# lanl-ansi/RestartSQP

Measured on NVIDIA B200. Metric: QP subproblems/sec, higher is better.
Workload: dtype f64

## Files before the change

restartsqp_b200/csrc/qp_kernel.cuh:

```cuda
#pragma once
#include <cuda_runtime.h>
#include <stdint.h>
#include "tma.cuh"

namespace sqpb200 {

#define QP_EPS 2.221e-16
#define QP_INFTY 1.0e20
#define QP_ZERO 1.0e-25
#define QP_BOUND_RELAX 1.0e4
#define QP_EPS_NUM (-1.0e3 * QP_EPS)
#define QP_EPS_DEN (1.0e3 * QP_EPS)
#define QP_EPS_FLIP (1.0e3 * QP_EPS)
#define QP_EPS_REG (1.0e3 * QP_EPS)
#define QP_EPS_LI (1.0e5 * QP_EPS)

enum { ST_OPTIMAL = 20, ST_INTERNAL = 21, ST_INFEASIBLE = 22, ST_UNBOUNDED = 23, ST_NOTINIT = 25, ST_HOMOTOPY = 28,
       ST_CAPACITY = 31  };
enum { MODE_COLD = 0, MODE_HOT_FIXED = 1, MODE_HOT_VARIED = 2,
       MODE_REINIT = 3  };
enum { FLAG_FLIPPING = 1, FLAG_RAMPING = 2, FLAG_DRIFT = 4, FLAG_KEEP_STATE = 8,
       FLAG_FORCE_GUESS = 16 ,
       FLAG_NO_CARRY = 32  };

// ... 60 lines not shown
    a.oW = o; if (a.large) o += a.cap * a.ld;
    if (a.large) o = (o + 15) & ~15;
    a.slice_doubles = o;
    a.state_doubles = a.oP + 2 * nV * nV;
    int p = 0;
    a.pAp = p; p += nV + 1; a.pAi = p; p += a.zA; a.pArp = p; p += nC + 1; a.pAci = p; p += a.zA; a.pAperm = p; p += a.zA;
    a.pHp = p; p += nV + 1; a.pHi = p; p += a.zH;
    a.pat_shorts = (p + 3) & ~3;
}

#ifdef __CUDACC__

__shared__ QPKernelArgs sA;
extern __shared__ __align__(128) double qp_smem[];

struct MinKey {
    double t;
    int pos;
};
__device__ __forceinline__ bool key_less(double t1, int p1, double t2, int p2) { return t1 < t2 || (t1 == t2 && p1 < p2); }

__device__ __forceinline__ double quot(double x, double d, double ri) {
    const double q0 = x * ri;
    const double r = __fma_rn(-q0, d, x);
    return __fma_rn(r, ri, q0);
}

#define QP_FN __noinline__
#define QP_U1 _Pragma("unroll 1")
#ifdef QP_PROFILE
#define PROF_T0 long long prof_t0_ = clock64();
#define PROF_RESET prof_t0_ = clock64();
#define PROF2_T0 long long prof_t2_ = clock64();
#define PROF2_ADD(i) do { long long t_ = clock64(); if (lane == 0 && sA.prof) atomicAdd((unsigned long long*)&sA.prof[i], (unsigned long long)(t_ - prof_t2_)); prof_t2_ = t_; } while (0)
#define PROF_ADD(i) do { long long t_ = clock64(); if (lane == 0 && sA.prof) atomicAdd((unsigned long long*)&sA.prof[i], (unsigned long long)(t_ - prof_t0_)); prof_t0_ = t_; } while (0)
#else
#define PROF_T0
#define PROF_RESET
#define PROF2_T0
#define PROF2_ADD(i) do { } while (0)
#define PROF_ADD(i) do { } while (0)
#endif
enum { PR_STEPDIR = 0, PR_RATIO = 1, PR_STEP = 2, PR_REMOVE = 3, PR_EXTEND = 4, PR_WVEC = 5, PR_ADD = 6, PR_REFAC_W = 7, PR_REFAC_M = 8,
       PR_REFAC_CHOL = 9, PR_DRIFT = 10, PR_ENSURE_LI = 11, PR_RSOLVE = 12, PR_SETUP = 13, PR_EPILOGUE = 14, PR_TOTAL = 15 };

template <int TEAM> struct PatIdx { typedef int type; };
template <> struct PatIdx<32> { typedef short type; };
template <> struct PatIdx<16> { typedef short type; };
template <> struct PatIdx<8> { typedef short type; };
template <int TEAM> __device__ __forceinline__ unsigned team_mask() {
    if (TEAM >= 32) return 0xffffffffu;
    return ((1u << (TEAM & 31)) - 1u) << ((threadIdx.x & 31) & ~(TEAM - 1));
}
__shared__ double* sSlice;
__shared__ int sClusterSize;
__shared__ uint32_t sPhase;
__shared__ __align__(8) uint64_t sFull[3];
__shared__ double sRedT[32];
__shared__ int sRedP[32];

#define QP_CTX                                                                                     \
    const int lane = (TEAM <= 32) ? (int)(threadIdx.x & (TEAM - 1)) : (int)threadIdx.x;            \
    double* const slice = (TEAM <= 32) ? qp_smem + (size_t)(threadIdx.x / TEAM) * sA.slice_doubles : sSlice; \
    int* const hdr = reinterpret_cast<int*>(slice);                                                \
    const int nV = sA.nV, nC = sA.nC, ld = sA.ld, cap = sA.cap;                                    \
    (void)lane; (void)hdr; (void)nV; (void)nC; (void)ld; (void)cap;
#define QP_PAT                                                                                     \
    const pidx* const pat = (TEAM <= 32)                                                           \
        ? reinterpret_cast<const pidx*>(qp_smem + (size_t)(blockDim.x / TEAM) * sA.slice_doubles) \
        : reinterpret_cast<const pidx*>(sA.gpat);

#define V_(name) (slice + sA.o##name)
#define S_(k) (reinterpret_cast<short*>(slice + sA.oS) + (k))
#define sB_ S_(0)
#define FR_ S_(nV)
#define posFR_ S_(2 * nV)
#define sC_ S_(3 * nV)
#define AC_ S_(3 * nV + nC)
#define posAC_ S_(3 * nV + 2 * nC)
#define R_(a_, b_) RT[(a_) * ld + (b_)]
#define T_(i, j) RT[(cap - 1 - (i)) * ld + (j)]
#define DOT_UNROLL _Pragma("unroll (TEAM <= 32 ? 1 : 8)")
#define SYNC() do { if (TEAM <= 32) __syncwarp(team_mask<TEAM>()); else __syncthreads(); } while (0)

template <int TEAM>
struct QPT {
    typedef typename PatIdx<TEAM>::type pidx;
    static __device__ __forceinline__ double H_row(const pidx* pat, const double* Hv, const double* v, int c) {
        const pidx *Hp = pat + sA.pHp, *Hi = pat + sA.pHi;
        const double reg = sA.is_lp ? QP_EPS_REG : 0.0;
        double s = 0.0;
        if (sA.has_H && !sA.is_lp) {
            int e1 = Hp[c + 1];
            QP_U1 for (int e = Hp[c]; e < e1; e++) s += Hv[e] * v[Hi[e]];
        }
        if (reg != 0.0) s += reg * v[c];
        return s;
    }
    static __device__ __forceinline__ double A_row(const pidx* pat, const double* Av, const double* v, int r) {
        const pidx *Arp = pat + sA.pArp, *Aci = pat + sA.pAci, *Aperm = pat + sA.pAperm;
        double s = 0.0;
        int k1 = Arp[r + 1];
        QP_U1 for (int k = Arp[r]; k < k1; k++) s += Av[Aperm[k]] * v[Aci[k]];
        return s;
    }
    static __device__ __forceinline__ double AT_col(const pidx* pat, const double* Av, const double* yc, int c) {
        const pidx *Ap = pat + sA.pAp, *Ai = pat + sA.pAi;
        double s = 0.0;
        int e1 = Ap[c + 1];
        QP_U1 for (int e = Ap[c]; e < e1; e++) s += Av[e] * yc[Ai[e]];
        return s;
    }
    static __device__ QP_FN void mulH(const double* v, double* out) {
        QP_CTX QP_PAT
        const double* Hv = V_(Hv);
        QP_U1 for (int c = lane; c < nV; c += TEAM) out[c] = H_row(pat, Hv, v, c);
        SYNC();
    }
    static __device__ QP_FN void mulH_noreg(const double* v, double* out) {
        QP_CTX QP_PAT
        const pidx *Hp = pat + sA.pHp, *Hi = pat + sA.pHi;
        const double* Hv = V_(Hv);
        const bool has_H = sA.has_H && !sA.is_lp;
        QP_U1 for (int c = lane; c < nV; c += TEAM) {
            double s = 0.0;
            if (has_H) {
                int e1 = Hp[c + 1];
                QP_U1 for (int e = Hp[c]; e < e1; e++) s += Hv[e] * v[Hi[e]];
            }
            out[c] = s;
        }
        SYNC();
    }
    static __device__ QP_FN void mulA(const double* v, double* out) {
        QP_CTX QP_PAT
        const double* Av = V_(Av);
        QP_U1 for (int r = lane; r < nC; r += TEAM) out[r] = A_row(pat, Av, v, r);
        SYNC();
    }
    static __device__ QP_FN void mulAT(const double* yc, double* out) {
        QP_CTX QP_PAT
        const double* Av = V_(Av);
        QP_U1 for (int c = lane; c < nV; c += TEAM) out[c] = AT_col(pat, Av, yc, c);
        SYNC();
    }
    static __device__ __forceinline__ double A_entry(const pidx* pat, const double* Av, int r, int c) {
        const pidx *Arp = pat + sA.pArp, *Aci = pat + sA.pAci, *Aperm = pat + sA.pAperm;
        double s = 0.0;
        int k1 = Arp[r + 1];
        QP_U1 for (int k = Arp[r]; k < k1; k++)
            if (Aci[k] == c) s += Av[Aperm[k]];
        return s;
    }

    static __device__ __forceinline__ MinKey team_min(double t, int pos) {
        const unsigned tm = team_mask<TEAM>();
        QP_U1 for (int o = (TEAM < 32 ? TEAM : 32) / 2; o > 0; o >>= 1) {
            double t2_ = __shfl_xor_sync(tm, t, o);
            int p2 = __shfl_xor_sync(tm, pos, o);
            if (key_less(t2_, p2, t, pos)) { t = t2_; pos = p2; }
        }
        if (TEAM > 32) {
            __syncthreads();
            if ((threadIdx.x & 31) == 0) { sRedT[threadIdx.x >> 5] = t; sRedP[threadIdx.x >> 5] = pos; }
            __syncthreads();
            t = sRedT[0]; pos = sRedP[0];
            QP_U1 for (int k = 1; k < TEAM / 32; k++)
                if (key_less(sRedT[k], sRedP[k], t, pos)) { t = sRedT[k]; pos = sRedP[k]; }
        }
        MinKey r; r.t = t; r.pos = pos;
        return r;
    }

    static __device__ __forceinline__ void givens(double a_, double b_, double& c, double& s, double& r) {
        if (a_ == 0.0) { c = 1.0; s = 0.0; r = b_; return; }
        double h = sqrt(a_ * a_ + b_ * b_);
        c = b_ / h; s = a_ / h; r = h;
    }

    static __device__ QP_FN void proj_column(int b) {
        QP_CTX
        double *t1 = V_(t1), *t2 = V_(t2);
        const double* Q = V_(Q);
        const short* posFR = posFR_;
        QP_U1 for (int i = lane; i < nV; i += TEAM) { int p = posFR[i]; t1[i] = (p >= 0) ? Q[p * ld + b] : 0.0; }
        SYNC();
        mulH(t1, t2);
    }
    static __device__ QP_FN int recompute_R() {
        QP_CTX
        const int nFR = hdr[0], nAC = hdr[1], nZ = nFR - nAC;
        if (nZ <= 0) return 0;
        double* RT = V_(RT);
        if (sA.is_lp) {
            double sr = sqrt(QP_EPS_REG);
            QP_U1 for (int k = lane; k < nZ * nZ; k += TEAM) { int a_ = k / nZ, b_ = k % nZ; R_(a_, b_) = (a_ == b_) ? sr : 0.0; }
            if constexpr (TEAM > 32) {
                double* W = V_(W);
                for (int k = lane; k < nZ * 64; k += TEAM) { const int a_ = k >> 6, c_ = k & 63; if (c_ < ld) W[(size_t)a_ * ld + c_] = (c_ == (a_ & 63)) ? 1.0 / sr : 0.0; }
            }
            SYNC();
            return 0;
        }
        if constexpr (TEAM > 32) return recompute_R_blocked();
        PROF_T0
        {
            QP_PAT
            const double *Q = V_(Q), *Hv = V_(Hv);
            double* Wc = V_(t1);
            const short *FR = FR_, *posFR = posFR_;
            const pidx *Hp = pat + sA.pHp, *Hi = pat + sA.pHi;
            const bool has_H = sA.has_H != 0;
            int CH = sA.nW / nFR;
            if (CH > nZ) CH = nZ;
            QP_U1 for (int b0 = 0; b0 < nZ; b0 += CH) {
                const int cw = (nZ - b0 < CH) ? nZ - b0 : CH;
                QP_U1 for (int e = lane; e < nFR * cw; e += TEAM) {
                    const int p = e / cw, bb = e - p * cw;
                    double s = 0.0;
                    if (has_H) {
                        const int c = FR[p], e1 = Hp[c + 1];
                        QP_U1 for (int h = Hp[c]; h < e1; h++) {
                            const int pr = posFR[Hi[h]];
                            s += Hv[h] * ((pr >= 0) ? Q[pr * ld + b0 + bb] : 0.0);
                        }
                    }
                    Wc[e] = s;
                }
                SYNC();
                QP_U1 for (int e = lane; e < (b0 + cw) * cw; e += TEAM) {
                    const int a_ = e / cw, bb = e - a_ * cw;
                    if (a_ <= b0 + bb) {
                        double s = 0.0;
                        QP_U1 for (int p = 0; p < nFR; p++) s += Q[p * ld + a_] * Wc[p * cw + bb];
                        R_(a_, b0 + bb) = s;
                    }
                }
                SYNC();
            }
        }
        PROF_ADD(PR_REFAC_M);
        QP_U1 for (int i = 0; i < nZ; i++) {
            QP_U1 for (int j = i + lane; j < nZ; j += TEAM) {
                double s = R_(i, j);
                DOT_UNROLL for (int k = 0; k < i; k++) s -= R_(k, i) * R_(k, j);
                R_(i, j) = s;
            }
            SYNC();
            double d = R_(i, i);
            SYNC();
            if (!(d > QP_ZERO)) return 1 + i;
            double dd = sqrt(d);
            QP_U1 for (int j = i + lane; j < nZ; j += TEAM) R_(i, j) = (j == i) ? dd : R_(i, j) / dd;
            QP_U1 for (int j = lane; j < i; j += TEAM) R_(i, j) = 0.0;
            SYNC();
        }
        PROF_ADD(PR_REFAC_CHOL);
        return 0;
    }

    static constexpr int LT_KC = 32, LT_STAGES = 3, LT_LD = 68, LT_NB = 64;
    static constexpr int LT_STAGE_DOUBLES = LT_KC * LT_LD;
    static constexpr int LT_D_LD = 65;
    static constexpr int LS_X = 0, LS_Y = LT_STAGES * LT_STAGE_DOUBLES, LS_D = 2 * LT_STAGES * LT_STAGE_DOUBLES,
                         LS_DI = LS_D + LT_NB * LT_D_LD, LS_RED = LS_DI + LT_NB * LT_D_LD, LS_TV = LS_RED + 8 * LT_NB,
                         LS_TOTAL = LS_TV + 2 * LT_NB;

    static __device__ __forceinline__ void large_sync() {
        asm volatile("fence.proxy.async;" ::: "memory");
        if (sClusterSize > 1) asm volatile("barrier.cluster.arrive.release.aligned;\n\tbarrier.cluster.wait.acquire.aligned;" ::: "memory");
        else __syncthreads();
    }
    static __device__ __forceinline__ void dmma(double (&c)[2], double a, double b) {
        asm volatile("mma.sync.aligned.m8n8k4.row.col.f64.f64.f64.f64 {%0,%1}, {%2}, {%3}, {%0,%1};" : "+d"(c[0]), "+d"(c[1]) : "d"(a), "d"(b));
    }
    template <int SIGN, bool TRI>
    static __device__ __forceinline__ void mma_tile(const double* X, int xw, const double* Y, int yw, int K, double* C, int na, int nb,
                                                    int ld, bool init_zero, int ga, int gb) {
        static_assert(TEAM == 512, "tile mapping assumes 16 warps");
        uint32_t ph = sPhase;
        double* Xs = qp_smem + LS_X;
        double* Ys = qp_smem + LS_Y;
        const int tid = threadIdx.x, warp = tid >> 5, l = tid & 31, g = l >> 2, t = l & 3;
        const int ra = (warp >> 2) * 16, cb = (warp & 3) * 16;
        double acc[2][2][2];
#pragma unroll
        for (int mi = 0; mi < 2; mi++)
#pragma unroll
            for (int ni = 0; ni < 2; ni++)
#pragma unroll
                for (int j = 0; j < 2; j++) {
                    const int a = ra + mi * 8 + g, b = cb + ni * 8 + t * 2 + j;
                    acc[mi][ni][j] = (!init_zero && a < na && b < nb && (!TRI || ga + a <= gb + b)) ? C[a * ld + b] : 0.0;
                }
        const int nch = (K + LT_KC - 1) / LT_KC;
        auto issue = [&](int chunk, int s) {
            const int rows = (K - chunk * LT_KC < LT_KC) ? K - chunk * LT_KC : LT_KC;
            if (l == 0) mbar_expect_tx(&sFull[s], (uint32_t)rows * (uint32_t)(xw + yw) * 8u);
            __syncwarp();
            if (l < rows) {
                const size_t kr = (size_t)(chunk * LT_KC + l) * ld;
                bulk_g2s(Xs + s * LT_STAGE_DOUBLES + l * LT_LD, X + kr, (uint32_t)xw * 8u, &sFull[s]);
                bulk_g2s(Ys + s * LT_STAGE_DOUBLES + l * LT_LD, Y + kr, (uint32_t)yw * 8u, &sFull[s]);
            }
        };
        if (warp == 0)
            for (int c = 0; c < LT_STAGES && c < nch; c++) issue(c, c);
        for (int c = 0; c < nch; c++) {
            const int s = c % LT_STAGES;
            while (!mbar_try_wait(&sFull[s], (ph >> s) & 1u)) {}
            ph ^= 1u << s;
            const int rows = (K - c * LT_KC < LT_KC) ? K - c * LT_KC : LT_KC;
            const double* xs = Xs + s * LT_STAGE_DOUBLES + ra + g;
            const double* ys = Ys + s * LT_STAGE_DOUBLES + cb + g;
            const int k4n = (rows + 3) >> 2;
#pragma unroll 2
            for (int k4 = 0; k4 < k4n; k4++) {
                const int kr = k4 * 4 + t;
                double a0 = xs[kr * LT_LD], a1 = xs[kr * LT_LD + 8], b0 = ys[kr * LT_LD], b1 = ys[kr * LT_LD + 8];
                if (kr >= rows) { a0 = 0.0; a1 = 0.0; b0 = 0.0; b1 = 0.0; }
                if (SIGN < 0) { a0 = -a0; a1 = -a1; }
                dmma(acc[0][0], a0, b0); dmma(acc[0][1], a0, b1); dmma(acc[1][0], a1, b0); dmma(acc[1][1], a1, b1);
            }
            __syncthreads();
            if (warp == 0 && c + LT_STAGES < nch) issue(c + LT_STAGES, s);
        }
#pragma unroll
        for (int mi = 0; mi < 2; mi++)
#pragma unroll
// ... 658 lines not shown
    }
    static __device__ QP_FN void bwd_solve_R_blocked(double* z, int n) {
        QP_CTX
        const double* RT = V_(RT);
        const double* W = V_(W);
        double* tv = qp_smem + LS_TV;
        const int tid = threadIdx.x, warp = tid >> 5, l = tid & 31;
        for (int i0 = ((n - 1) >> 6) << 6; i0 >= 0; i0 -= LT_NB) {
            const int nb = (n - i0 < LT_NB) ? n - i0 : LT_NB, i1 = i0 + nb;
            double dreg[4][2];
#pragma unroll
            for (int q = 0; q < 4; q++) {
                const int r = warp + (TEAM / 32) * q;
#pragma unroll
                for (int h = 0; h < 2; h++) { const int cc = r + l + 32 * h; dreg[q][h] = (r < nb && cc < nb) ? W[(size_t)(i0 + r) * ld + cc] : 0.0; }
            }
            {
                double s4[4] = {0.0, 0.0, 0.0, 0.0};
#pragma unroll 2
                for (int k = i1 + 2 * l; k < n; k += 64) {
                    const double zk = z[k], zk1 = (k + 1 < n) ? z[k + 1] : 0.0;
#pragma unroll
                    for (int q = 0; q < 4; q++) {
                        const int r = warp + (TEAM / 32) * q;
                        if (r < nb) { const double2 v = *reinterpret_cast<const double2*>(&R_(i0 + r, k)); s4[q] += v.x * zk + ((k + 1 < n) ? v.y * zk1 : 0.0); }
                    }
                }
#pragma unroll
                for (int q = 0; q < 4; q++) {
                    double sq = s4[q];
#pragma unroll
                    for (int o = 16; o > 0; o >>= 1) sq += __shfl_xor_sync(0xffffffffu, sq, o);
                    const int r = warp + (TEAM / 32) * q;
                    if (l == 0 && r < nb) tv[r] = z[i0 + r] - sq;
                }
            }
            __syncthreads();
#pragma unroll
            for (int q = 0; q < 4; q++) {
                const int r = warp + (TEAM / 32) * q;
                double s = 0.0;
#pragma unroll
                for (int h = 0; h < 2; h++) { const int cc = r + l + 32 * h; if (r < nb && cc < nb) s += dreg[q][h] * tv[cc]; }
#pragma unroll
                for (int o = 16; o > 0; o >>= 1) s += __shfl_xor_sync(0xffffffffu, s, o);
                if (l == 0 && r < nb) z[i0 + r] = s;
            }
            __syncthreads();
        }
    }
    static __device__ QP_FN void extend_Dinv(int b, double rho) {
        QP_CTX
        const double* RT = V_(RT);
        double* W = V_(W);
        const int i0 = (b >> 6) << 6, c = b - i0, tid = threadIdx.x;
        if (tid < c) {
            double s = 0.0;
            for (int q = tid; q < c; q++) s += W[(size_t)(i0 + tid) * ld + q] * R_(i0 + q, b);
            W[(size_t)(i0 + tid) * ld + c] = -s / rho;
        } else if (tid == c) W[(size_t)(i0 + c) * ld + c] = 1.0 / rho;
        __syncthreads();
    }
    static __device__ QP_FN int extend_R(int check_curvature) {
        QP_CTX
        const int nFR = hdr[0], nAC = hdr[1], nZ = nFR - nAC, b = nZ - 1;
        double *RT = V_(RT), *w = V_(w);
        if (sA.is_lp) {
            QP_U1 for (int a_ = lane; a_ < b; a_ += TEAM) { R_(a_, b) = 0.0; R_(b, a_) = 0.0; }
            if (lane == 0) R_(b, b) = sqrt(QP_EPS_REG);
            SYNC();
            if constexpr (TEAM > 32) extend_Dinv(b, sqrt(QP_EPS_REG));
            return 1;
        }
        const double *Q = V_(Q), *t2 = V_(t2);
        const short* FR = FR_;
        proj_column(b);
        if constexpr (TEAM > 32) {
            double* tmp = V_(a);
            for (int p = lane; p < nFR; p += TEAM) tmp[p] = t2[FR[p]];
            SYNC();
            col_sums_auto(sA.oQ, nFR, 0, b + 1, sA.oa, sA.ow, false);
        } else
        {
        QP_U1 for (int a_ = lane; a_ <= b; a_ += TEAM) {
            double s = 0.0;
            DOT_UNROLL for (int p = 0; p < nFR; p++) s += Q[p * ld + a_] * t2[FR[p]];
            w[a_] = s;
        }
        SYNC();
        }
        if constexpr (TEAM > 32) fwd_solve_R_blocked(w, b, b);
        else {
        double* rinv = V_(dy);
        QP_U1 for (int k = lane; k < b; k += TEAM) rinv[k] = 1.0 / R_(k, k);
        SYNC();
        QP_U1 for (int k = 0; k < b; k++) {
            double rk = quot(w[k], R_(k, k), rinv[k]);
            SYNC();
            if (lane == 0) R_(k, b) = rk;
            QP_U1 for (int i = k + 1 + lane; i < b; i += TEAM) w[i] -= R_(k, i) * rk;
            SYNC();
        }
        }
        double rho2 = w[b];
        if constexpr (TEAM > 32) {
            double part = 0.0;
            for (int k = lane; k < b; k += TEAM) part += R_(k, b) * R_(k, b);
            rho2 -= team_sum(part);
        } else
        {
        DOT_UNROLL for (int k = 0; k < b; k++) rho2 -= R_(k, b) * R_(k, b);
        }
        int ok = check_curvature ? (rho2 > QP_EPS_FLIP) : (rho2 > QP_ZERO);
        SYNC();
        if (!ok) return 0;
        if (lane == 0) R_(b, b) = sqrt(rho2);
        QP_U1 for (int a_ = lane; a_ < b; a_ += TEAM) R_(b, a_) = 0.0;
        SYNC();
        if constexpr (TEAM > 32) extend_Dinv(b, sqrt(rho2));
        return 1;
    }

    static __device__ QP_FN void constraint_w(int c, double& wz2, double& a2) {
        QP_CTX QP_PAT
        const int nFR = hdr[0], nAC = hdr[1], nZ = nFR - nAC;
        double *a = V_(a), *w = V_(w);
        const double *Q = V_(Q), *Av = V_(Av);
        const short* FR = FR_;
        QP_U1 for (int p = lane; p < nFR; p += TEAM) a[p] = A_entry(pat, Av, c, FR[p]);
        SYNC();
        if constexpr (TEAM > 32) {
            col_sums_auto(sA.oQ, nFR, 0, nFR, sA.oa, sA.ow, false);
            double s2p = 0.0, z2p = 0.0;
            for (int p = lane; p < nFR; p += TEAM) s2p += a[p] * a[p];
            for (int j = lane; j < nZ; j += TEAM) z2p += w[j] * w[j];
            a2 = team_sum(s2p); wz2 = team_sum(z2p);
            SYNC();
            return;
        }
        QP_U1 for (int j = lane; j < nFR; j += TEAM) {
            double s = 0.0;
            DOT_UNROLL for (int p = 0; p < nFR; p++) s += Q[p * ld + j] * a[p];
            w[j] = s;
        }
        SYNC();
        double s2 = 0.0, z2 = 0.0;
        DOT_UNROLL for (int p = 0; p < nFR; p++) s2 += a[p] * a[p];
        DOT_UNROLL for (int j = 0; j < nZ; j++) z2 += w[j] * w[j];
        wz2 = z2; a2 = s2;
        SYNC();
    }
    static __device__ QP_FN double rotation_chain(int cnt) {
        QP_CTX
        double *t2 = V_(t2), *t3 = V_(t3);
        const double* w = V_(w);
        QP_U1 for (int j = lane; j + 1 < cnt; j += TEAM) {
            double S = w[0] * w[0];
            bool anyprev = false;
            DOT_UNROLL for (int k = 1; k <= j; k++) { anyprev = anyprev || (w[k - 1] != 0.0); S = S + w[k] * w[k]; }
            const double a = anyprev ? sqrt(S) : w[j];
            if (a == 0.0) { t2[j] = 1.0; t3[j] = 0.0; }
            else { const double h = sqrt(S + w[j + 1] * w[j + 1]); t2[j] = w[j + 1] / h; t3[j] = a / h; }
        }
        double r;
        {
            const int j = cnt - 1;
            double S = w[0] * w[0];
            bool anyprev = false;
            DOT_UNROLL for (int k = 1; k <= j; k++) { anyprev = anyprev || (w[k - 1] != 0.0); S = S + w[k] * w[k]; }
            r = anyprev ? sqrt(S) : w[j];
        }
        SYNC();
        return r;
    }
    static __device__ QP_FN void add_constraint(int c, int status, bool carry_R = false) {
        QP_CTX
        const int nFR = hdr[0], nAC = hdr[1], nZ = nFR - nAC;
        double *Q = V_(Q), *RT = V_(RT);
        const double *t2 = V_(t2), *t3 = V_(t3), *w = V_(w);
        double r = rotation_chain(nZ);
        if constexpr (TEAM > 32) {
            rot_rows_auto(sA.oQ, nFR, nZ, sA.ot2, sA.ot3);
            if (carry_R) update_R_after_add(nZ);
        } else
        {
        QP_U1 for (int p = lane; p < nFR; p += TEAM) {
            double* q = Q + p * ld;
            double qa = q[0];
            QP_U1 for (int j = 0; j + 1 < nZ; j++) {
                double cs = t2[j], sn = t3[j], qb = q[j + 1];
                q[j] = cs * qa - sn * qb;
                qa = sn * qa + cs * qb;
            }
            if (nZ > 0) q[nZ - 1] = qa;
        }
        }
        QP_U1 for (int j = lane; j < nFR; j += TEAM) T_(nAC, j) = (j > nZ - 1) ? w[j] : ((j == nZ - 1) ? r : 0.0);
        if (lane == 0) { AC_[nAC] = (short)c; posAC_[c] = (short)nAC; sC_[c] = (short)status; hdr[1] = nAC + 1; }
        SYNC();
    }
    static __device__ QP_FN void removal_chain_regs(int i0, int c0) {
        QP_CTX
        const int nFR = hdr[0], nAC = hdr[1];
        double *Q = V_(Q), *RT = V_(RT), *t2 = V_(t2), *t3 = V_(t3);
        const unsigned tm = team_mask<TEAM>();
        constexpr int W = TEAM <= 32 ? TEAM : 32;
        const bool own = lane >= i0 && lane < nAC;
        double tb = own ? T_(lane, c0 - i0 + 1) : 0.0;
        QP_U1 for (int i = i0; i < nAC; i++) {
            const int cL = c0 - i;
            const bool act = own && lane >= i;
            const double ta = act ? T_(lane, cL) : 0.0;
            double cs, sn, r;
            givens(__shfl_sync(tm, ta, i, W), __shfl_sync(tm, tb, i, W), cs, sn, r);
            if (act) {
                T_(lane, cL + 1) = sn * ta + cs * tb;
                tb = cs * ta - sn * tb;
                if (lane == i) { T_(lane, cL) = 0.0; t2[i - i0] = cs; t3[i - i0] = sn; }
            }
        }
        SYNC();
        QP_U1 for (int p = lane; p < nFR; p += TEAM) {
            double* q = Q + p * ld;
            double qb = q[c0 - i0 + 1];
            QP_U1 for (int i = i0; i < nAC; i++) {
                const int cL = c0 - i;
                const double cs = t2[i - i0], sn = t3[i - i0], qa = q[cL];
                q[cL + 1] = sn * qa + cs * qb;
                qb = cs * qa - sn * qb;
            }
            q[c0 - nAC + 1] = qb;
        }
    }
    static __device__ QP_FN void remove_constraint(int c) {
        QP_CTX
        const int nFR = hdr[0], nAC = hdr[1];
        double *Q = V_(Q), *RT = V_(RT);
        short *AC = AC_, *posAC = posAC_;
        const int k = posAC[c];
        SYNC();
        if (TEAM <= 32 && nAC <= TEAM) {
            if (k + 1 < nAC) removal_chain_regs(k + 1, nFR - 1);
        } else {
        QP_U1 for (int i = k + 1; i < nAC; i++) {
            int cL = nFR - 1 - i;
            double cs, sn, r;
            givens(T_(i, cL), T_(i, cL + 1), cs, sn, r);
            SYNC();
            QP_U1 for (int ii = i + lane; ii < nAC; ii += TEAM) {
                double ta = T_(ii, cL), tb = T_(ii, cL + 1);
                T_(ii, cL) = (ii == i) ? 0.0 : cs * ta - sn * tb;
                T_(ii, cL + 1) = sn * ta + cs * tb;
            }
            if constexpr (TEAM > 32) {
                if (lane == 0) { V_(t2)[i - k - 1] = cs; V_(t3)[i - k - 1] = -sn; }
            } else
            {
            QP_U1 for (int p = lane; p < nFR; p += TEAM) {
                double qa = Q[p * ld + cL], qb = Q[p * ld + cL + 1];
                Q[p * ld + cL] = cs * qa - sn * qb;
                Q[p * ld + cL + 1] = sn * qa + cs * qb;
            }
            }
            SYNC();
        }
        }
        if constexpr (TEAM > 32) rot_rows_auto(sA.oQ, nFR, nAC - k, sA.ot2, sA.ot3, nFR - 1 - k, -1);
        QP_U1 for (int j = lane; j < nFR; j += TEAM)
            QP_U1 for (int i = k + 1; i < nAC; i++) T_(i - 1, j) = T_(i, j);
        SYNC();
        if (lane == 0) {
            QP_U1 for (int i = k + 1; i < nAC; i++) { AC[i - 1] = AC[i]; posAC[AC[i - 1]] = (short)(i - 1); }
            sC_[c] = 0; posAC[c] = -1; hdr[1] = nAC - 1;
        }
        SYNC();
    }
    static __device__ QP_FN double bound_w(int v) {
        QP_CTX
        const int nFR = hdr[0], nAC = hdr[1], nZ = nFR - nAC, p = posFR_[v];
        double* w = V_(w);
        const double* Q = V_(Q);
        QP_U1 for (int j = lane; j < nFR; j += TEAM) w[j] = Q[p * ld + j];
        SYNC();
        if constexpr (TEAM > 32) {
            double z2p = 0.0;
            for (int j = lane; j < nZ; j += TEAM) z2p += w[j] * w[j];
            const double z2s = team_sum(z2p);
            SYNC();
            return z2s;
        }
        double z2 = 0.0;
        DOT_UNROLL for (int j = 0; j < nZ; j++) z2 += w[j] * w[j];
        SYNC();
        return z2;
    }
    static __device__ QP_FN void add_bound(int v, int status, bool carry_R = false) {
        QP_CTX
        const int nFR = hdr[0], nAC = hdr[1], nZ = nFR - nAC;
        double *Q = V_(Q), *RT = V_(RT);
        const double *t2 = V_(t2), *t3 = V_(t3);
        short *FR = FR_, *posFR = posFR_;
        const int p = posFR[v];
        rotation_chain(nFR);
        if constexpr (TEAM > 32) {
            rot_rows_auto(sA.oQ, nFR, nFR, sA.ot2, sA.ot3);
            if (carry_R) update_R_after_add(nZ);
        } else
        {
        QP_U1 for (int pp = lane; pp < nFR; pp += TEAM) {
            double* q = Q + pp * ld;
            double qa = q[0];
            QP_U1 for (int j = 0; j + 1 < nFR; j++) {
                double cs = t2[j], sn = t3[j], qb = q[j + 1];
                q[j] = cs * qa - sn * qb;
                qa = sn * qa + cs * qb;
            }
            q[nFR - 1] = qa;
        }
        }
        QP_U1 for (int i = lane; i < nAC; i += TEAM) {
            int j0 = nFR - 2 - i; if (j0 < nZ - 1) j0 = nZ - 1; if (j0 < 0) j0 = 0;
            double ta = T_(i, j0);
            QP_U1 for (int j = j0; j + 1 < nFR; j++) {
                double cs = t2[j], sn = t3[j], tb = T_(i, j + 1);
                T_(i, j) = cs * ta - sn * tb;
                ta = sn * ta + cs * tb;
            }
            T_(i, nFR - 1) = ta;
        }
        SYNC();
        const int last = nFR - 1;
        if (p != last) {
            QP_U1 for (int j = lane; j < nFR - 1; j += TEAM) Q[p * ld + j] = Q[last * ld + j];
            if (lane == 0) { short vl = FR[last]; FR[p] = vl; posFR[vl] = (short)p; }
        }
        if (lane == 0) { posFR[v] = -1; sB_[v] = (short)status; hdr[0] = nFR - 1; }
        SYNC();
    }
    static __device__ QP_FN int remove_bound(int v) {
        QP_CTX QP_PAT
        int nFR = hdr[0];
        const int nAC = hdr[1];
        if (nFR + 1 > cap) return 1;
        double *Q = V_(Q), *RT = V_(RT);
        const double* Av = V_(Av);
        const pidx *Ap = pat + sA.pAp, *Ai = pat + sA.pAi;
        const short* AC = AC_;
        SYNC();
        QP_U1 for (int j = lane; j < nFR; j += TEAM) { Q[nFR * ld + j] = 0.0; Q[j * ld + nFR] = 0.0; }
        QP_U1 for (int i = lane; i < nAC; i += TEAM) {
            int r = AC[i];
            double s = 0.0;
            int e1 = Ap[v + 1];
            QP_U1 for (int e = Ap[v]; e < e1; e++)
                if (Ai[e] == r) s += Av[e];
            T_(i, nFR) = s;
        }
        if (lane == 0) { Q[nFR * ld + nFR] = 1.0; FR_[nFR] = (short)v; posFR_[v] = (short)nFR; sB_[v] = 0; hdr[0] = nFR + 1; if (nFR + 1 > hdr[6]) hdr[6] = nFR + 1; }
        nFR++;
        SYNC();
        if (TEAM <= 32 && nAC <= TEAM) {
            if (nAC > 0) { removal_chain_regs(0, nFR - 2); SYNC(); }
            return 0;
        }
        QP_U1 for (int i = 0; i < nAC; i++) {
            int cL = nFR - 2 - i;
            double cs, sn, r;
            givens(T_(i, cL), T_(i, cL + 1), cs, sn, r);
            SYNC();
            QP_U1 for (int ii = i + lane; ii < nAC; ii += TEAM) {
                double ta = T_(ii, cL), tb = T_(ii, cL + 1);
                T_(ii, cL) = (ii == i) ? 0.0 : cs * ta - sn * tb;
                T_(ii, cL + 1) = sn * ta + cs * tb;
            }
            if constexpr (TEAM > 32) {
// ... 10 lines not shown
        }
        if constexpr (TEAM > 32) rot_rows_auto(sA.oQ, nFR, nAC + 1, sA.ot2, sA.ot3, nFR - 1, -1);
        return 0;
    }

    static __device__ QP_FN void solve_T(double* b, double* v) {
        QP_CTX
        const int nFR = hdr[0], nAC = hdr[1];
        const double* RT = V_(RT);
        if constexpr (TEAM > 32) { solve_T_blocked(b, v); return; }
        if (TEAM <= 32 && nAC <= TEAM) {
            const bool act = lane < nAC;
            double bk = act ? b[lane] : 0.0;
            const double piv = act ? T_(lane, nFR - 1 - lane) : 1.0, ri = 1.0 / piv;
            QP_U1 for (int i = 0; i < nAC; i++) {
                const int d = nFR - 1 - i;
                const double tkd = (lane > i && act) ? T_(lane, d) : 0.0;
                const double vi = __shfl_sync(team_mask<TEAM>(), quot(bk, piv, ri), i, TEAM <= 32 ? TEAM : 32);
                if (lane == i) v[d] = vi;
                if (lane > i && act) bk -= tkd * vi;
            }
            SYNC();
            return;
        }
        double* rinv = V_(dAx);
        QP_U1 for (int i = lane; i < nAC; i += TEAM) rinv[i] = 1.0 / T_(i, nFR - 1 - i);
        SYNC();
        QP_U1 for (int i = 0; i < nAC; i++) {
            int d = nFR - 1 - i;
            double vi = quot(b[i], T_(i, d), rinv[i]);
            SYNC();
            if (lane == 0) v[d] = vi;
            QP_U1 for (int k = i + 1 + lane; k < nAC; k += TEAM) b[k] -= T_(k, d) * vi;
            SYNC();
        }
    }
    static __device__ QP_FN void solve_Tt(double* r, double* u) {
        QP_CTX
        const int nFR = hdr[0], nAC = hdr[1];
        const double* RT = V_(RT);
        if constexpr (TEAM > 32) { solve_Tt_blocked(r, u); return; }
        if (TEAM <= 32 && nAC <= TEAM) {
            const bool act = lane < nAC;
            double rk = act ? r[nFR - 1 - lane] : 0.0;
            const double piv = act ? T_(lane, nFR - 1 - lane) : 1.0, ri = 1.0 / piv;
            QP_U1 for (int i = nAC - 1; i >= 0; i--) {
                const double tik = (lane < i) ? T_(i, nFR - 1 - lane) : 0.0;
                const double ui = __shfl_sync(team_mask<TEAM>(), quot(rk, piv, ri), i, TEAM <= 32 ? TEAM : 32);
                if (lane == i) u[i] = ui;
                if (lane < i) rk -= tik * ui;
            }
            SYNC();
            return;
        }
        double* rinv = V_(dAx);
        QP_U1 for (int i = lane; i < nAC; i += TEAM) rinv[i] = 1.0 / T_(i, nFR - 1 - i);
        SYNC();
        QP_U1 for (int i = nAC - 1; i >= 0; i--) {
            int d = nFR - 1 - i;
            double ui = quot(r[d], T_(i, d), rinv[i]);
            SYNC();
            if (lane == 0) u[i] = ui;
            QP_U1 for (int k = lane; k < i; k += TEAM) { int dk = nFR - 1 - k; r[dk] -= T_(i, dk) * ui; }
            SYNC();
        }
    }

    static __device__ QP_FN void step_direction(const double* dgvec, const double* dxFX, double* dbAC) {
        QP_CTX QP_PAT
        const int nT = nV + nC;
        const int nFR = hdr[0], nAC = hdr[1], nZ = nFR - nAC;
        double *dx = V_(dx), *dy = V_(dy), *dAx = V_(dAx), *t1 = V_(t1), *t3 = V_(t3), *yv = V_(yv), *zv = V_(zv);
        const double *Q = V_(Q), *RT = V_(RT), *Av = V_(Av), *Hv = V_(Hv);
        const short *sB = sB_, *FR = FR_, *AC = AC_;
        QP_U1 for (int i = lane; i < nV; i += TEAM) dx[i] = (sB[i] != 0) ? dxFX[i] : 0.0;
        SYNC();
        if (nAC > 0) {
            QP_U1 for (int i = lane; i < nAC; i += TEAM) t3[i] = dbAC[i] - A_row(pat, Av, dx, AC[i]);
            SYNC();
            solve_T(t3, yv);
            if constexpr (TEAM > 32) row_sums_auto(sA.oQ, nFR, nZ, nFR, sA.oyv, sA.odx, true, false);
            else
            {
            QP_U1 for (int p = lane; p < nFR; p += TEAM) {
                double s = 0.0;
                DOT_UNROLL for (int j = nZ; j < nFR; j++) s += Q[p * ld + j] * yv[j];
                dx[FR[p]] = s;
            }
            SYNC();
            }
        }
        if (nZ > 0) {
            mulH(dx, t1);
            if constexpr (TEAM > 32) {
                for (int p = lane; p < nFR; p += TEAM) { const int v = FR[p]; yv[p] = t1[v] + dgvec[v]; }
                SYNC();
                col_sums_auto(sA.oQ, nFR, 0, nZ, sA.oyv, sA.ozv, true);
            } else
            {
            double* rinv = V_(dy);
            QP_U1 for (int j = lane; j < nZ; j += TEAM) {
                double s = 0.0;
                DOT_UNROLL for (int p = 0; p < nFR; p++) { int v = FR[p]; s += Q[p * ld + j] * (t1[v] + dgvec[v]); }
                zv[j] = -s;
                rinv[j] = 1.0 / R_(j, j);
            }
            SYNC();
            }
            PROF2_T0
            if constexpr (TEAM > 32) {
                fwd_solve_R_blocked(zv, nZ, -1);
                bwd_solve_R_blocked(zv, nZ);
                PROF2_ADD(PR_RSOLVE);
            } else {
                const double* rinv = V_(dy);
                QP_U1 for (int k = 0; k < nZ; k++) {
                    double uk = quot(zv[k], R_(k, k), rinv[k]);
                    SYNC();
                    if (lane == 0) zv[k] = uk;
                    QP_U1 for (int i = k + 1 + lane; i < nZ; i += TEAM) zv[i] -= R_(k, i) * uk;
                    SYNC();
                }
                QP_U1 for (int k = nZ - 1; k >= 0; k--) {
                    double zk = quot(zv[k], R_(k, k), rinv[k]);
                    SYNC();
                    if (lane == 0) zv[k] = zk;
                    QP_U1 for (int i = lane; i < k; i += TEAM) zv[i] -= R_(i, k) * zk;
                    SYNC();
                }
                PROF2_ADD(PR_RSOLVE);
            }
            if constexpr (TEAM > 32) row_sums_auto(sA.oQ, nFR, 0, nZ, sA.ozv, sA.odx, true, true);
            else
            {
            QP_U1 for (int p = lane; p < nFR; p += TEAM) {
                double s = 0.0;
                DOT_UNROLL for (int j = 0; j < nZ; j++) s += Q[p * ld + j] * zv[j];
                dx[FR[p]] += s;
            }
            SYNC();
            }
        }
        QP_U1 for (int i = lane; i < nV; i += TEAM) t1[i] = H_row(pat, Hv, dx, i) + dgvec[i];
        QP_U1 for (int i = lane; i < nT; i += TEAM) dy[i] = 0.0;
        SYNC();
        if (nAC > 0) {
            if constexpr (TEAM > 32) {
                for (int p = lane; p < nFR; p += TEAM) zv[p] = t1[FR[p]];
                SYNC();
                col_sums_auto(sA.oQ, nFR, nZ, nFR, sA.ozv, sA.oyv, false);
            } else
            {
            QP_U1 for (int j = nZ + lane; j < nFR; j += TEAM) {
                double s = 0.0;
                DOT_UNROLL for (int p = 0; p < nFR; p++) s += Q[p * ld + j] * t1[FR[p]];
                yv[j] = s;
            }
            SYNC();
            }
            solve_Tt(yv, t3);
            QP_U1 for (int i = lane; i < nAC; i += TEAM) dy[nV + AC[i]] = t3[i];
            SYNC();
            QP_U1 for (int i = lane; i < nV; i += TEAM) if (sB[i] != 0) dy[i] = t1[i] - AT_col(pat, Av, dy + nV, i);
        } else {
            QP_U1 for (int i = lane; i < nV; i += TEAM) if (sB[i] != 0) dy[i] = t1[i];
        }
        QP_U1 for (int r = lane; r < nC; r += TEAM) dAx[r] = A_row(pat, Av, dx, r);
        SYNC();
    }

    static __device__ QP_FN void stationarity_gradient_tail() {
        QP_CTX QP_PAT
        double* g = V_(g);
        const double *t1 = V_(t1), *y = V_(y), *Av = V_(Av);
        QP_U1 for (int i = lane; i < nV; i += TEAM) g[i] = AT_col(pat, Av, y + nV, i) + y[i] - t1[i];
        SYNC();
    }
    static __device__ QP_FN void stationarity_gradient() {
        QP_CTX
        mulH(V_(x), V_(t1));
        stationarity_gradient_tail();
    }
    static __device__ QP_FN void drift_correction() {
        QP_CTX QP_PAT
        double *x = V_(x), *y = V_(y), *Ax = V_(Ax), *lb = V_(lb), *ub = V_(ub), *lbA = V_(lbA), *ubA = V_(ubA), *t1 = V_(t1);
        const double *Av = V_(Av), *Hv = V_(Hv);
        const short *sB = sB_, *sC = sC_;
        QP_U1 for (int i = lane; i < nV; i += TEAM) {
            int s = sB[i]; double xi = x[i];
            if (s < 0) { lb[i] = xi; if (ub[i] < xi) ub[i] = xi; if (y[i] < 0) y[i] = 0.0; }
            else if (s > 0) { ub[i] = xi; if (lb[i] > xi) lb[i] = xi; if (y[i] > 0) y[i] = 0.0; }
            else { if (lb[i] > xi) lb[i] = xi; if (ub[i] < xi) ub[i] = xi; y[i] = 0.0; }
            t1[i] = H_row(pat, Hv, x, i);
        }
        QP_U1 for (int i = lane; i < nC; i += TEAM) {
            int s = sC[i]; double ax = A_row(pat, Av, x, i);
            Ax[i] = ax;
            if (s < 0) { lbA[i] = ax; if (ubA[i] < ax) ubA[i] = ax; if (y[nV + i] < 0) y[nV + i] = 0.0; }
            else if (s > 0) { ubA[i] = ax; if (lbA[i] > ax) lbA[i] = ax; if (y[nV + i] > 0) y[nV + i] = 0.0; }
            else { if (lbA[i] > ax) lbA[i] = ax; if (ubA[i] < ax) ubA[i] = ax; y[nV + i] = 0.0; }
        }
        SYNC();
        stationarity_gradient_tail();
    }
    static __device__ QP_FN void ramping() {
        QP_CTX QP_PAT
        double *x = V_(x), *y = V_(y), *Ax = V_(Ax), *lb = V_(lb), *ub = V_(ub), *lbA = V_(lbA), *ubA = V_(ubA), *t1 = V_(t1);
        const double *Av = V_(Av), *Hv = V_(Hv);
        const short *sB = sB_, *sC = sC_;
        const int ramp_offset = hdr[2];
        const int nRamp = nV + nC + nC + nV;
        const double r0 = 0.5, r1 = 1.0;
        QP_U1 for (int i = lane; i < nV; i += TEAM) {
            double tP = (double)((i + ramp_offset) % nRamp) / (double)(nRamp - 1);
            double rP = (1.0 - tP) * r0 + tP * r1;
            double tD = (double)((nV + nC + i + ramp_offset) % nRamp) / (double)(nRamp - 1);
            double rD = (1.0 - tD) * r0 + tD * r1;
            double xi = x[i];
            double sca = fabs(xi) > 1.0 ? fabs(xi) : 1.0;
            int s = sB[i];
            if (s >= 0) lb[i] = xi - sca * rP;
            if (s <= 0) ub[i] = xi + sca * rP;
            if (s < 0) { lb[i] = xi; y[i] = rD; }
            if (s > 0) { ub[i] = xi; y[i] = -rD; }
            if (s == 0) y[i] = 0.0;
            t1[i] = H_row(pat, Hv, x, i);
        }
        QP_U1 for (int i = lane; i < nC; i += TEAM) {
            double tP = (double)((nV + i + ramp_offset) % nRamp) / (double)(nRamp - 1);
            double rP = (1.0 - tP) * r0 + tP * r1;
            double tD = (double)((nV + nC + nV + i + ramp_offset) % nRamp) / (double)(nRamp - 1);
            double rD = (1.0 - tD) * r0 + tD * r1;
            double ax = A_row(pat, Av, x, i);
            Ax[i] = ax;
            double sca = fabs(ax) > 1.0 ? fabs(ax) : 1.0;
            int s = sC[i];
            if (s >= 0) lbA[i] = ax - sca * rP;
            if (s <= 0) ubA[i] = ax + sca * rP;
            if (s < 0) { lbA[i] = ax; y[nV + i] = rD; }
            if (s > 0) { ubA[i] = ax; y[nV + i] = -rD; }
// ... 650 lines not shown
```

Baseline: 10.56 million.

## Add load-ahead dot helper, gather operands once, shuffle-based triangular solves for small teams

Introduces an osum/dot helper for small (warp-or-smaller) teams that issues the next four index, value and operand loads before accumulating the current products. This hides shared-memory latency in sparse row/column products and dense dot loops. Gathered vectors (t2[FR], t1[FR]+dg) are staged into contiguous scratch once instead of being re-gathered inside every dot product. Triangular forward/backward solves with dimension at most TEAM now keep values in registers and broadcast pivots with warp shuffles instead of a SYNC per step. The trade-offs are extra register pressure and extra synchronisation for the staging steps.

```diff
diff --git a/restartsqp_b200/csrc/qp_kernel.cuh b/restartsqp_b200/csrc/qp_kernel.cuh
--- a/restartsqp_b200/csrc/qp_kernel.cuh
+++ b/restartsqp_b200/csrc/qp_kernel.cuh
@@ -166,34 +166,79 @@
 #define T_(i, j) RT[(cap - 1 - (i)) * ld + (j)]
 #define DOT_UNROLL _Pragma("unroll (TEAM <= 32 ? 1 : 8)")
 #define SYNC() do { if (TEAM <= 32) __syncwarp(team_mask<TEAM>()); else __syncthreads(); } while (0)
+#if defined(QP_WPS) && QP_WPS >= 32
+#define QP_SUM_AHEAD 0
+#else
+#define QP_SUM_AHEAD 1
+#endif
 
 template <int TEAM>
 struct QPT {
     typedef typename PatIdx<TEAM>::type pidx;
+    template <bool SUB = false, class IX, class LA, class LB>
+    static __device__ __forceinline__ double osum(double s, int k0, int k1, IX ix, LA la, LB lb) {
+        int k = k0;
+        if constexpr (TEAM <= 32 && QP_SUM_AHEAD) {
+            if (k0 + 4 <= k1) {
+                auto i0 = ix(k), i1 = ix(k + 1), i2 = ix(k + 2), i3 = ix(k + 3);
+                double a0 = la(k, i0), a1 = la(k + 1, i1), a2 = la(k + 2, i2), a3 = la(k + 3, i3);
+                double b0 = lb(k, i0), b1 = lb(k + 1, i1), b2 = lb(k + 2, i2), b3 = lb(k + 3, i3);
+                k += 4;
+                QP_U1 for (; k + 4 <= k1; k += 4) {
+                    const double p0 = a0 * b0, p1 = a1 * b1, p2 = a2 * b2, p3 = a3 * b3;
+                    i0 = ix(k); i1 = ix(k + 1); i2 = ix(k + 2); i3 = ix(k + 3);
+                    a0 = la(k, i0); a1 = la(k + 1, i1); a2 = la(k + 2, i2); a3 = la(k + 3, i3);
+                    b0 = lb(k, i0); b1 = lb(k + 1, i1); b2 = lb(k + 2, i2); b3 = lb(k + 3, i3);
+                    if (SUB) { s -= p0; s -= p1; s -= p2; s -= p3; } else { s += p0; s += p1; s += p2; s += p3; }
+                }
+                const double p0 = a0 * b0, p1 = a1 * b1, p2 = a2 * b2, p3 = a3 * b3;
+                if (SUB) { s -= p0; s -= p1; s -= p2; s -= p3; } else { s += p0; s += p1; s += p2; s += p3; }
+            }
+        }
+        QP_U1 for (; k < k1; k++) {
+            const auto i = ix(k);
+            const double p = la(k, i) * lb(k, i);
+            if (SUB) s -= p; else s += p;
+        }
+        return s;
+    }
+    template <bool SUB = false>
+    static __device__ QP_FN double dot(double s, int k0, int k1, const double* a, int sa, const double* b, int sb) {
+        return osum<SUB>(s, k0, k1, [](int k) { return k; }, [=](int k, int) { return a[k * sa]; }, [=](int k, int) { return b[k * sb]; });
+    }
+
     static __device__ __forceinline__ double H_row(const pidx* pat, const double* Hv, const double* v, int c) {
         const pidx *Hp = pat + sA.pHp, *Hi = pat + sA.pHi;
         const double reg = sA.is_lp ? QP_EPS_REG : 0.0;
         double s = 0.0;
         if (sA.has_H && !sA.is_lp) {
-            int e1 = Hp[c + 1];
-            QP_U1 for (int e = Hp[c]; e < e1; e++) s += Hv[e] * v[Hi[e]];
+            const int e1 = Hp[c + 1];
+            if constexpr (TEAM > 32) { QP_U1 for (int e = Hp[c]; e < e1; e++) s += Hv[e] * v[Hi[e]]; }
+            else s = osum(s, Hp[c], e1, [=](int e) { return (int)Hi[e]; }, [=](int e, int) { return Hv[e]; }, [=](int, int i) { return v[i]; });
         }
         if (reg != 0.0) s += reg * v[c];
         return s;
     }
     static __device__ __forceinline__ double A_row(const pidx* pat, const double* Av, const double* v, int r) {
         const pidx *Arp = pat + sA.pArp, *Aci = pat + sA.pAci, *Aperm = pat + sA.pAperm;
-        double s = 0.0;
-        int k1 = Arp[r + 1];
-        QP_U1 for (int k = Arp[r]; k < k1; k++) s += Av[Aperm[k]] * v[Aci[k]];
-        return s;
+        const int k1 = Arp[r + 1];
+        if constexpr (TEAM > 32) {
+            double s = 0.0;
+            QP_U1 for (int k = Arp[r]; k < k1; k++) s += Av[Aperm[k]] * v[Aci[k]];
+            return s;
+        }
+        return osum(0.0, Arp[r], k1, [=](int k) { return make_int2(Aperm[k], Aci[k]); }, [=](int, int2 i) { return Av[i.x]; },
+                    [=](int, int2 i) { return v[i.y]; });
     }
     static __device__ __forceinline__ double AT_col(const pidx* pat, const double* Av, const double* yc, int c) {
         const pidx *Ap = pat + sA.pAp, *Ai = pat + sA.pAi;
-        double s = 0.0;
-        int e1 = Ap[c + 1];
-        QP_U1 for (int e = Ap[c]; e < e1; e++) s += Av[e] * yc[Ai[e]];
-        return s;
+        const int e1 = Ap[c + 1];
+        if constexpr (TEAM > 32) {
+            double s = 0.0;
+            QP_U1 for (int e = Ap[c]; e < e1; e++) s += Av[e] * yc[Ai[e]];
+            return s;
+        }
+        return osum(0.0, Ap[c], e1, [=](int e) { return (int)Ai[e]; }, [=](int e, int) { return Av[e]; }, [=](int, int i) { return yc[i]; });
     }
     static __device__ QP_FN void mulH(const double* v, double* out) {
         QP_CTX QP_PAT
@@ -326,9 +371,7 @@
         PROF_ADD(PR_REFAC_M);
         QP_U1 for (int i = 0; i < nZ; i++) {
             QP_U1 for (int j = i + lane; j < nZ; j += TEAM) {
-                double s = R_(i, j);
-                DOT_UNROLL for (int k = 0; k < i; k++) s -= R_(k, i) * R_(k, j);
-                R_(i, j) = s;
+                R_(i, j) = dot<true>(R_(i, j), 0, i, &R_(0, i), ld, &R_(0, j), ld);
             }
             SYNC();
             double d = R_(i, i);
@@ -1153,15 +1196,25 @@
             col_sums_auto(sA.oQ, nFR, 0, b + 1, sA.oa, sA.ow, false);
         } else
         {
-        QP_U1 for (int a_ = lane; a_ <= b; a_ += TEAM) {
-            double s = 0.0;
-            DOT_UNROLL for (int p = 0; p < nFR; p++) s += Q[p * ld + a_] * t2[FR[p]];
-            w[a_] = s;
-        }
+        double* tmp = V_(a);
+        QP_U1 for (int p = lane; p < nFR; p += TEAM) tmp[p] = t2[FR[p]];
+        SYNC();
+        QP_U1 for (int a_ = lane; a_ <= b; a_ += TEAM) w[a_] = dot(0.0, 0, nFR, Q + a_, ld, tmp, 1);
         SYNC();
         }
         if constexpr (TEAM > 32) fwd_solve_R_blocked(w, b, b);
-        else {
+        else if (b <= TEAM) {
+            const bool act = lane < b;
+            double wk = act ? w[lane] : 0.0;
+            const double piv = act ? R_(lane, lane) : 1.0, ri = 1.0 / piv;
+            QP_U1 for (int k = 0; k < b; k++) {
+                const double rkl = (lane > k && act) ? R_(k, lane) : 0.0;
+                const double rk = __shfl_sync(team_mask<TEAM>(), quot(wk, piv, ri), k, TEAM <= 32 ? TEAM : 32);
+                if (lane == k) R_(k, b) = rk;
+                if (lane > k && act) wk -= rkl * rk;
+            }
+            SYNC();
+        } else {
         double* rinv = V_(dy);
         QP_U1 for (int k = lane; k < b; k += TEAM) rinv[k] = 1.0 / R_(k, k);
         SYNC();
@@ -1180,7 +1233,7 @@
             rho2 -= team_sum(part);
         } else
         {
-        DOT_UNROLL for (int k = 0; k < b; k++) rho2 -= R_(k, b) * R_(k, b);
+        rho2 = dot<true>(rho2, 0, b, &R_(0, b), ld, &R_(0, b), ld);
         }
         int ok = check_curvature ? (rho2 > QP_EPS_FLIP) : (rho2 > QP_ZERO);
         SYNC();
@@ -1209,16 +1262,10 @@
             SYNC();
             return;
         }
-        QP_U1 for (int j = lane; j < nFR; j += TEAM) {
-            double s = 0.0;
-            DOT_UNROLL for (int p = 0; p < nFR; p++) s += Q[p * ld + j] * a[p];
-            w[j] = s;
-        }
-        SYNC();
-        double s2 = 0.0, z2 = 0.0;
-        DOT_UNROLL for (int p = 0; p < nFR; p++) s2 += a[p] * a[p];
-        DOT_UNROLL for (int j = 0; j < nZ; j++) z2 += w[j] * w[j];
-        wz2 = z2; a2 = s2;
+        QP_U1 for (int j = lane; j < nFR; j += TEAM) w[j] = dot(0.0, 0, nFR, Q + j, ld, a, 1);
+        SYNC();
+        wz2 = dot(0.0, 0, nZ, w, 1, w, 1);
+        a2 = dot(0.0, 0, nFR, a, 1, a, 1);
         SYNC();
     }
     static __device__ QP_FN double rotation_chain(int cnt) {
@@ -1360,8 +1407,7 @@
             SYNC();
             return z2s;
         }
-        double z2 = 0.0;
-        DOT_UNROLL for (int j = 0; j < nZ; j++) z2 += w[j] * w[j];
+        const double z2 = dot(0.0, 0, nZ, w, 1, w, 1);
         SYNC();
         return z2;
     }
@@ -1538,11 +1584,7 @@
             if constexpr (TEAM > 32) row_sums_auto(sA.oQ, nFR, nZ, nFR, sA.oyv, sA.odx, true, false);
             else
             {
-            QP_U1 for (int p = lane; p < nFR; p += TEAM) {
-                double s = 0.0;
-                DOT_UNROLL for (int j = nZ; j < nFR; j++) s += Q[p * ld + j] * yv[j];
-                dx[FR[p]] = s;
-            }
+            QP_U1 for (int p = lane; p < nFR; p += TEAM) dx[FR[p]] = dot(0.0, nZ, nFR, Q + p * ld, 1, yv, 1);
             SYNC();
             }
         }
@@ -1554,11 +1596,11 @@
                 col_sums_auto(sA.oQ, nFR, 0, nZ, sA.oyv, sA.ozv, true);
             } else
             {
+            QP_U1 for (int p = lane; p < nFR; p += TEAM) { const int v = FR[p]; yv[p] = t1[v] + dgvec[v]; }
+            SYNC();
             double* rinv = V_(dy);
             QP_U1 for (int j = lane; j < nZ; j += TEAM) {
-                double s = 0.0;
-                DOT_UNROLL for (int p = 0; p < nFR; p++) { int v = FR[p]; s += Q[p * ld + j] * (t1[v] + dgvec[v]); }
-                zv[j] = -s;
+                zv[j] = -dot(0.0, 0, nFR, Q + j, ld, yv, 1);
                 rinv[j] = 1.0 / R_(j, j);
             }
             SYNC();
@@ -1567,6 +1609,25 @@
             if constexpr (TEAM > 32) {
                 fwd_solve_R_blocked(zv, nZ, -1);
                 bwd_solve_R_blocked(zv, nZ);
+                PROF2_ADD(PR_RSOLVE);
+            } else if (nZ <= TEAM) {
+                const bool act = lane < nZ;
+                double zk = act ? zv[lane] : 0.0;
+                const double piv = act ? R_(lane, lane) : 1.0, ri = 1.0 / piv;
+                QP_U1 for (int k = 0; k < nZ; k++) {
+                    const double rkl = (lane > k && act) ? R_(k, lane) : 0.0;
+                    const double uk = __shfl_sync(team_mask<TEAM>(), quot(zk, piv, ri), k, TEAM <= 32 ? TEAM : 32);
+                    if (lane == k) zk = uk;
+                    if (lane > k && act) zk -= rkl * uk;
+                }
+                QP_U1 for (int k = nZ - 1; k >= 0; k--) {
+                    const double rlk = (lane < k) ? R_(lane, k) : 0.0;
+                    const double zkk = __shfl_sync(team_mask<TEAM>(), quot(zk, piv, ri), k, TEAM <= 32 ? TEAM : 32);
+                    if (lane == k) zk = zkk;
+                    if (lane < k) zk -= rlk * zkk;
+                }
+                if (act) zv[lane] = zk;
+                SYNC();
                 PROF2_ADD(PR_RSOLVE);
             } else {
                 const double* rinv = V_(dy);
@@ -1589,11 +1650,7 @@
             if constexpr (TEAM > 32) row_sums_auto(sA.oQ, nFR, 0, nZ, sA.ozv, sA.odx, true, true);
             else
             {
-            QP_U1 for (int p = lane; p < nFR; p += TEAM) {
-                double s = 0.0;
-                DOT_UNROLL for (int j = 0; j < nZ; j++) s += Q[p * ld + j] * zv[j];
-                dx[FR[p]] += s;
-            }
+            QP_U1 for (int p = lane; p < nFR; p += TEAM) dx[FR[p]] += dot(0.0, 0, nZ, Q + p * ld, 1, zv, 1);
             SYNC();
             }
         }
@@ -1607,11 +1664,9 @@
                 col_sums_auto(sA.oQ, nFR, nZ, nFR, sA.ozv, sA.oyv, false);
             } else
             {
-            QP_U1 for (int j = nZ + lane; j < nFR; j += TEAM) {
-                double s = 0.0;
-                DOT_UNROLL for (int p = 0; p < nFR; p++) s += Q[p * ld + j] * t1[FR[p]];
-                yv[j] = s;
-            }
+            QP_U1 for (int p = lane; p < nFR; p += TEAM) zv[p] = t1[FR[p]];
+            SYNC();
+            QP_U1 for (int j = nZ + lane; j < nFR; j += TEAM) yv[j] = dot(0.0, 0, nFR, Q + j, ld, zv, 1);
             SYNC();
             }
             solve_Tt(yv, t3);
```

Result: slower. 9.594 million (median of 6 runs) (-9.2%).
